# Atif-Anwer/SHMGAN

Hardware: AMD Instinct MI355X
Metric: images/sec (gen+disc train_step) (higher is better)
Workload: dtype f32; 1 GPU; SHMGAN train_step 256x256 5-view, batch 8/GPU, filter_size 64, fp32 (BASELINE configs[1]); global_batch=8, image_size=256, parallelism=dp1, losses_finite=True

## Files before the change

shmgan_amd/csrc/imgloss.hip:

```cpp
#include "common.h"

#define Y2R_V_R 1.13988303f
#define Y2R_U_G -0.394642334f
#define Y2R_V_G -0.58062185f
#define Y2R_U_B 2.03206185f

constexpr int NSUM = 19;
constexpr int WIN = SHM_SSIM_WIN;
constexpr int TILE = 16;
constexpr int HALO = TILE + WIN - 1;

struct ImgArgs {
    const float* gen_rgb;
    const float* cyc_rgb;
    const float* cyc_y;
    const float* cbcr;
    const float* orig[5];
    const float* ds[5];
    int flags;
    float style_factor;
    double* loss;
    float* dgen_y;
    float* dcyc_y;
    double* sums;
    unsigned* mm;
    float* gd;
    double* ssim_sum;
    float* gcoef;
    double* rsum;
    int* argpos;
    float* dmaps;
    int batch, s;
};

__device__ __forceinline__ unsigned f2ord(float f) {
    unsigned u = __float_as_uint(f);
    return (u & 0x80000000u) ? ~u : (u | 0x80000000u);
}
__device__ __forceinline__ float ord2f(unsigned u) {
    return __uint_as_float((u & 0x80000000u) ? (u & 0x7fffffffu) : ~u);
}

__global__ __launch_bounds__(256) void img_pass_a(const ImgArgs a) {
    const int b = blockIdx.y, B = a.batch;
    const size_t npix = (size_t)a.s * a.s;
    const float invB = 1.0f / B, inv3n = 1.0f / (3.0f * (float)npix);
    double sm[NSUM];
#pragma unroll
    for (int i = 0; i < NSUM; ++i) sm[i] = 0.0;
    float mn[10], mx[10];
#pragma unroll
    for (int i = 0; i < 10; ++i) { mn[i] = 3.0e38f; mx[i] = -3.0e38f; }

    for (size_t p = (size_t)blockIdx.x * 256 + threadIdx.x; p < npix; p += (size_t)gridDim.x * 256) {
        const size_t bp = (size_t)b * npix + p;
        const float u = a.cbcr[bp * 2], v = a.cbcr[bp * 2 + 1];
        {
            float g = 0.f;
#pragma unroll
            for (int c = 0; c < 3; ++c) {
                float d = a.gen_rgb[bp * 3 + c] - a.orig[4][bp * 3 + c];
                sm[0] += fabs((double)d);
                g += (d > 0.f) ? 1.f : (d < 0.f ? -1.f : 0.f);
            }
            a.dgen_y[bp] = 10.0f * 0.2f * invB * inv3n * g;
        }
#pragma unroll
        for (int k = 0; k < 5; ++k) {
            const size_t ip = ((size_t)k * B + b) * npix + p;
            float g = 0.f;
#pragma unroll
            for (int c = 0; c < 3; ++c) {
                float d = a.cyc_rgb[ip * 3 + c] - a.orig[k][bp * 3 + c];
                sm[1 + k] += fabs((double)d);
                g += (d > 0.f) ? 1.f : (d < 0.f ? -1.f : 0.f);
            }
            float grad = 10.0f * (k == 4 ? 10.0f : 0.2f) * invB * inv3n * g;
            const float y = a.cyc_y[ip];
            mn[k] = fminf(mn[k], fminf(y, fminf(u, v)));
            mx[k] = fmaxf(mx[k], fmaxf(y, fmaxf(u, v)));
            const float d0 = a.ds[k][bp * 3], d1 = a.ds[k][bp * 3 + 1], d2 = a.ds[k][bp * 3 + 2];
            mn[5 + k] = fminf(mn[5 + k], fminf(d0, fminf(d1, d2)));
            mx[5 + k] = fmaxf(mx[5 + k], fmaxf(d0, fmaxf(d1, d2)));
            if (k == 4) {
                const float e0 = y - a.ds[0][bp * 3], e1 = u - a.ds[0][bp * 3 + 1], e2 = v - a.ds[0][bp * 3 + 2];
                sm[6] += (double)e0 * e0 + (double)e1 * e1 + (double)e2 * e2;
                grad += 10.0f * invB * 2.0f * e0 * inv3n;
                sm[7] += (double)y * y;  sm[8] += (double)y * u;  sm[9] += (double)y * v;
                sm[10] += (double)u * u; sm[11] += (double)u * v; sm[12] += (double)v * v;
                sm[13] += (double)d0 * d0; sm[14] += (double)d0 * d1; sm[15] += (double)d0 * d2;
                sm[16] += (double)d1 * d1; sm[17] += (double)d1 * d2; sm[18] += (double)d2 * d2;
            }
            a.dcyc_y[ip] = grad;
        }
    }
#pragma unroll
    for (int i = 0; i < NSUM; ++i) {
        double s = shm_block_sum<256>(sm[i]);
        if (threadIdx.x == 0) atomicAdd(&a.sums[(size_t)b * NSUM + i], s);
    }
#pragma unroll
    for (int i = 0; i < 10; ++i) {
        float lo = shm_wave_min(mn[i]), hi = shm_wave_max(mx[i]);
        if ((threadIdx.x & 63) == 0) {
            atomicMin(&a.mm[((size_t)b * 10 + i) * 2], f2ord(lo));
            atomicMax(&a.mm[((size_t)b * 10 + i) * 2 + 1], f2ord(hi));
        }
    }
}

__global__ void img_pass_b(const ImgArgs a) {
    if (blockIdx.x != 0 || threadIdx.x != 0) return;
    const double npix = (double)a.s * a.s;
    for (int b = 0; b < a.batch; ++b) {
        const double* sm = a.sums + (size_t)b * NSUM;
        for (int i = 0; i < 6; ++i) a.loss[i] += sm[i] / (3.0 * npix);
        a.loss[16] += sm[6] / (3.0 * npix);
        double D[6];
        for (int i = 0; i < 6; ++i) D[i] = (sm[7 + i] - sm[13 + i]) / npix;
        double sq = D[0] * D[0] + D[3] * D[3] + D[5] * D[5] + 2.0 * (D[1] * D[1] + D[2] * D[2] + D[4] * D[4]);
        a.loss[17] += (double)a.style_factor * sq / 9.0;
        a.gd[b * 4 + 0] = (float)D[0];
        a.gd[b * 4 + 1] = (float)D[1];
        a.gd[b * 4 + 2] = (float)D[2];
    }
}

__global__ void img_style_grad(const ImgArgs a) {
    const size_t npix = (size_t)a.s * a.s;
    size_t idx = (size_t)blockIdx.x * blockDim.x + threadIdx.x;
    if (idx >= (size_t)a.batch * npix) return;
    const int b = (int)(idx / npix);
    const size_t ip = (size_t)4 * a.batch * npix + idx;
    const float y = a.cyc_y[ip], u = a.cbcr[idx * 2], v = a.cbcr[idx * 2 + 1];
    const float coef = 1000.0f / a.batch * 4.0f * a.style_factor / (9.0f * (float)npix);
    a.dcyc_y[ip] += coef * (a.gd[b * 4] * y + a.gd[b * 4 + 1] * u + a.gd[b * 4 + 2] * v);
}

__device__ __forceinline__ float cyc_val(const ImgArgs& a, int b, int k, int c, size_t p, size_t npix) {
    if (c == 0) return a.cyc_y[((size_t)k * a.batch + b) * npix + p];
    return a.cbcr[((size_t)b * npix + p) * 2 + (c - 1)];
}

__global__ __launch_bounds__(256) void ssim_fwd_kernel(const ImgArgs a) {
    __shared__ float xs[HALO][HALO + 1], ys[HALO][HALO + 1];
    __shared__ float hx[HALO][TILE + 1], hy[HALO][TILE + 1], hxy[HALO][TILE + 1], hsq[HALO][TILE + 1];
    __shared__ float w1[WIN];
    const int S = a.s, HO = S - WIN + 1;
    const int tiles_x = (HO + TILE - 1) / TILE;
    const int ty = blockIdx.x / tiles_x, tx = blockIdx.x % tiles_x;
    const int bk = blockIdx.y, b = bk / 5, k = bk % 5, c = blockIdx.z;
    const size_t npix = (size_t)S * S;
    const float xmn = ord2f(a.mm[((size_t)b * 10 + k) * 2]), xmx = ord2f(a.mm[((size_t)b * 10 + k) * 2 + 1]);
    const float ymn = ord2f(a.mm[((size_t)b * 10 + 5 + k) * 2]), ymx = ord2f(a.mm[((size_t)b * 10 + 5 + k) * 2 + 1]);
    const float xr = xmx > xmn ? xmx - xmn : 0.f, yr = ymx > ymn ? ymx - ymn : 0.f;
    if (threadIdx.x == 0) shm_ssim_gauss1d(w1);
    const int oy0 = ty * TILE, ox0 = tx * TILE;
    for (int i = threadIdx.x; i < HALO * HALO; i += 256) {
        int r = i / HALO, cc = i % HALO;
        int yy = oy0 + r, xx = ox0 + cc;
        float xv = 0.f, yv = 0.f;
        if (yy < S && xx < S) {
            size_t p = (size_t)yy * S + xx;
            float xraw = cyc_val(a, b, k, c, p, npix);
            float yraw = a.ds[k][((size_t)b * npix + p) * 3 + c];
            xv = xr > 0.f ? (xraw - xmn) / xr : 0.f;
            yv = yr > 0.f ? (yraw - ymn) / yr : 0.f;
        }
        xs[r][cc] = xv;
        ys[r][cc] = yv;
    }
    __syncthreads();
    for (int i = threadIdx.x; i < HALO * TILE; i += 256) {
        const int r = i / TILE, cx = i % TILE;
        float rx = 0.f, ry = 0.f, rxy = 0.f, rsq = 0.f;
        for (int j = 0; j < WIN; ++j) {
            float xv = xs[r][cx + j], yv = ys[r][cx + j], w = w1[j];
            rx += w * xv;
            ry += w * yv;
            rxy += w * xv * yv;
            rsq += w * (xv * xv + yv * yv);
        }
        hx[r][cx] = rx;
        hy[r][cx] = ry;
        hxy[r][cx] = rxy;
        hsq[r][cx] = rsq;
    }
    __syncthreads();
    const int ly = threadIdx.x / TILE, lx = threadIdx.x % TILE;
    const int oy = oy0 + ly, ox = ox0 + lx;
    double sval = 0.0;
    if (oy < HO && ox < HO) {
        float mx_ = 0.f, my_ = 0.f, exy = 0.f, esq = 0.f;
        for (int i = 0; i < WIN; ++i) {
            mx_ += w1[i] * hx[ly + i][lx];
            my_ += w1[i] * hy[ly + i][lx];
            exy += w1[i] * hxy[ly + i][lx];
            esq += w1[i] * hsq[ly + i][lx];
        }
        const float c1 = 0.0025f, c2 = 0.0225f;
        const float A1 = 2.f * mx_ * my_ + c1, B1 = mx_ * mx_ + my_ * my_ + c1;
        const float A2 = 2.f * exy - 2.f * mx_ * my_ + c2, B2 = esq - mx_ * mx_ - my_ * my_ + c2;
        const float l = A1 / B1, cs = A2 / B2;
        sval = (double)(l * cs);
        const float dmx = cs * (2.f * my_ * B1 - A1 * 2.f * mx_) / (B1 * B1) + l * (-2.f * my_ * B2 + A2 * 2.f * mx_) / (B2 * B2);
        const float dexy = l * 2.f / B2;
        const float desq = -l * A2 / (B2 * B2);
        const size_t no = (size_t)HO * HO;
        float* dm = a.dmaps + ((size_t)bk * 3 + c) * 3 * no + (size_t)oy * HO + ox;
        dm[0] = dmx;
        dm[no] = dexy;
        dm[2 * no] = desq;
    }
    sval = shm_block_sum<256>(sval);
    if (threadIdx.x == 0) atomicAdd(&a.ssim_sum[bk], sval);
}

__global__ void ssim_finalize_kernel(const ImgArgs a) {
    if (blockIdx.x != 0 || threadIdx.x != 0) return;
    const int HO = a.s - WIN + 1;
    const double cnt = 3.0 * (double)HO * HO;
    for (int b = 0; b < a.batch; ++b)
        for (int k = 0; k < 5; ++k) {
            double ssim = a.ssim_sum[b * 5 + k] / cnt;
            bool fl = (a.flags >> k) & 1;
            a.loss[6 + k] += ssim;
            double sl = fl ? 0.0 : -log((1.0 + ssim) / 2.0);
            a.loss[11 + k] += sl;
            double coef = 10.0 * (k == 4 ? 2.0 : 0.2) / a.batch;
            a.gcoef[b * 5 + k] = fl ? 0.f : (float)(coef * (-1.0 / (1.0 + ssim)) / cnt);
        }
}

__global__ __launch_bounds__(256) void ssim_bwd_kernel(const ImgArgs a) {
    __shared__ float d0[HALO][HALO + 1], d1[HALO][HALO + 1], d2[HALO][HALO + 1];
    __shared__ float h0[HALO][TILE + 1], h1[HALO][TILE + 1], h2[HALO][TILE + 1];
    __shared__ float w1[WIN];
    const int S = a.s, HO = S - WIN + 1;
    const int tiles_x = (S + TILE - 1) / TILE;
    const int ty = blockIdx.x / tiles_x, tx = blockIdx.x % tiles_x;
    const int bk = blockIdx.y, b = bk / 5, k = bk % 5, c = blockIdx.z;
    const float gco = a.gcoef[bk];
    if (gco == 0.f) return;
    const size_t npix = (size_t)S * S, no = (size_t)HO * HO;
    const float xmn = ord2f(a.mm[((size_t)b * 10 + k) * 2]), xmx = ord2f(a.mm[((size_t)b * 10 + k) * 2 + 1]);
    const float ymn = ord2f(a.mm[((size_t)b * 10 + 5 + k) * 2]), ymx = ord2f(a.mm[((size_t)b * 10 + 5 + k) * 2 + 1]);
    const float xr = xmx > xmn ? xmx - xmn : 0.f, yr = ymx > ymn ? ymx - ymn : 0.f;
    if (threadIdx.x == 0) shm_ssim_gauss1d(w1);
    const int qy0 = ty * TILE, qx0 = tx * TILE;
    const float* dm = a.dmaps + ((size_t)bk * 3 + c) * 3 * no;
    for (int i = threadIdx.x; i < HALO * HALO; i += 256) {
        int r = i / HALO, cc = i % HALO;
        int py = qy0 - (WIN - 1) + r, px = qx0 - (WIN - 1) + cc;
        float v0 = 0.f, v1 = 0.f, v2 = 0.f;
        if (py >= 0 && py < HO && px >= 0 && px < HO) {
            size_t o = (size_t)py * HO + px;
            v0 = dm[o];
            v1 = dm[no + o];
            v2 = dm[2 * no + o];
        }
        d0[r][cc] = v0;
        d1[r][cc] = v1;
        d2[r][cc] = v2;
    }
    __syncthreads();
    for (int i = threadIdx.x; i < HALO * TILE; i += 256) {
        const int rr = i / TILE, cx = i % TILE;
        float r0 = 0.f, r1 = 0.f, r2 = 0.f;
        for (int j = 0; j < WIN; ++j) {
            const int cc = cx + (WIN - 1) - j;
            const float w = w1[j];
            r0 += w * d0[rr][cc];
            r1 += w * d1[rr][cc];
            r2 += w * d2[rr][cc];
        }
        h0[rr][cx] = r0;
        h1[rr][cx] = r1;
        h2[rr][cx] = r2;
    }
    __syncthreads();
    const int ly = threadIdx.x / TILE, lx = threadIdx.x % TILE;
    const int qy = qy0 + ly, qx = qx0 + lx;
    double sdx = 0.0, sdxr = 0.0;
    if (qy < S && qx < S) {
        float g0 = 0.f, g1 = 0.f, g2 = 0.f;
        for (int i = 0; i < WIN; ++i) {
            const int rr = ly + (WIN - 1) - i;
            g0 += w1[i] * h0[rr][lx];
            g1 += w1[i] * h1[rr][lx];
            g2 += w1[i] * h2[rr][lx];
        }
        const size_t p = (size_t)qy * S + qx;
        const float xraw = cyc_val(a, b, k, c, p, npix);
        const float yraw = a.ds[k][((size_t)b * npix + p) * 3 + c];
        const float xv = xr > 0.f ? (xraw - xmn) / xr : 0.f;
        const float yv = yr > 0.f ? (yraw - ymn) / yr : 0.f;
        const float dx = gco * (g0 + yv * g1 + 2.f * xv * g2);
        sdx = (double)dx;
        sdxr = (double)dx * (double)xv;
        if (c == 0 && xr > 0.f) {
            a.dcyc_y[((size_t)k * a.batch + b) * npix + p] += dx / xr;
            if (xraw == xmn) a.argpos[bk * 2] = (int)p;
            if (xraw == xmx) a.argpos[bk * 2 + 1] = (int)p;
        }
    }
    sdx = shm_block_sum<256>(sdx);
    sdxr = shm_block_sum<256>(sdxr);
    if (threadIdx.x == 0) {
        atomicAdd(&a.rsum[bk * 2], sdx);
        atomicAdd(&a.rsum[bk * 2 + 1], sdxr);
    }
}

__global__ void ssim_minmax_kernel(const ImgArgs a) {
    int bk = blockIdx.x * blockDim.x + threadIdx.x;
    if (bk >= a.batch * 5) return;
    const int b = bk / 5, k = bk % 5;
    if (a.gcoef[bk] == 0.f) return;
    const float xmn = ord2f(a.mm[((size_t)b * 10 + k) * 2]), xmx = ord2f(a.mm[((size_t)b * 10 + k) * 2 + 1]);
    if (!(xmx > xmn)) return;
    const double inv = 1.0 / ((double)xmx - (double)xmn);
    const double sdx = a.rsum[bk * 2], sdxr = a.rsum[bk * 2 + 1];
    const size_t npix = (size_t)a.s * a.s;
    float* dy = a.dcyc_y + ((size_t)k * a.batch + b) * npix;
    const int pmin = a.argpos[bk * 2], pmax = a.argpos[bk * 2 + 1];
    if (pmin >= 0) dy[pmin] += (float)(-(sdx - sdxr) * inv);
    if (pmax >= 0) dy[pmax] += (float)(-sdxr * inv);
}

static size_t align256(size_t v) { return (v + 255) & ~(size_t)255; }

struct WsPlan {
    size_t sums, mm, gd, ssim_sum, gcoef, rsum, argpos, dmaps, total, zero_bytes;
};

static WsPlan plan_ws(int batch, int s) {
    WsPlan w;
    size_t off = 0;
    w.sums = off;     off = align256(off + (size_t)batch * NSUM * 8);
    w.ssim_sum = off; off = align256(off + (size_t)batch * 5 * 8);
    w.rsum = off;     off = align256(off + (size_t)batch * 10 * 8);
    w.gd = off;       off = align256(off + (size_t)batch * 4 * 4);
    w.gcoef = off;    off = align256(off + (size_t)batch * 5 * 4);
    w.zero_bytes = off;
    w.mm = off;       off = align256(off + (size_t)batch * 20 * 4);
    w.argpos = off;   off = align256(off + (size_t)batch * 10 * 4);
    w.dmaps = off;
    int ho = s - WIN + 1;
    off = align256(off + (size_t)batch * 5 * 3 * 3 * ho * ho * 4);
    w.total = off;
    return w;
}

extern "C" size_t shm_image_losses_workspace(int batch, int s) {
    if (s < WIN) return 0;
    return plan_ws(batch, s).total;
}

__global__ void init_mm_kernel(unsigned* mm, int n) {
    int i = blockIdx.x * blockDim.x + threadIdx.x;
    if (i < n) mm[i] = (i & 1) ? 0u : 0xffffffffu;
}

extern "C" int shm_image_losses(const float* gen_rgb, const float* cyc_rgb, const float* cyc_y, const float* cbcr,
                                const float* const* orig, const float* const* ds, int flags_mask, float style_factor,
                                double* loss, float* dgen_y, float* dcyc_y, void* ws, size_t ws_bytes, int batch, int s,
                                void* stream) {
    SHM_REQUIRE(s >= WIN, SHM_E_SHAPE, "shm_image_losses: image size %d < 11 (ssim window)", s);
    SHM_REQUIRE(batch > 0 && batch * 5 <= 65535, SHM_E_SHAPE, "shm_image_losses: bad batch %d", batch);
    WsPlan w = plan_ws(batch, s);
    SHM_REQUIRE(ws && ws_bytes >= w.total, SHM_E_WORKSPACE, "shm_image_losses: workspace %zu < %zu bytes", ws_bytes, w.total);
    hipStream_t st = (hipStream_t)stream;
    char* base = (char*)ws;
    ImgArgs a{};
    a.gen_rgb = gen_rgb;
    a.cyc_rgb = cyc_rgb;
    a.cyc_y = cyc_y;
    a.cbcr = cbcr;
    for (int i = 0; i < 5; ++i) {
        a.orig[i] = orig[i];
        a.ds[i] = ds[i];
    }
    a.flags = flags_mask;
    a.style_factor = style_factor;
    a.loss = loss;
    a.dgen_y = dgen_y;
    a.dcyc_y = dcyc_y;
    a.sums = (double*)(base + w.sums);
    a.mm = (unsigned*)(base + w.mm);
    a.gd = (float*)(base + w.gd);
    a.ssim_sum = (double*)(base + w.ssim_sum);
    a.gcoef = (float*)(base + w.gcoef);
    a.rsum = (double*)(base + w.rsum);
    a.argpos = (int*)(base + w.argpos);
    a.dmaps = (float*)(base + w.dmaps);
    a.batch = batch;
    a.s = s;

    int r = shm_zero(base, w.zero_bytes, stream);
    if (r) return r;
    r = shm_zero(loss, 32 * sizeof(double), stream);
    if (r) return r;
    hipError_t e = hipMemsetAsync(a.argpos, 0xff, (size_t)batch * 10 * 4, st);
    SHM_REQUIRE(e == hipSuccess, SHM_E_HIP, "shm_image_losses: memset: %s", hipGetErrorString(e));
    hipLaunchKernelGGL(init_mm_kernel, dim3(shm_cdiv(batch * 20, 64)), dim3(64), 0, st, a.mm, batch * 20);
    SHM_LAUNCH_CHECK("shm_image_losses(init)");

    const size_t npix = (size_t)s * s;
    const int nblk = shm_grid_cap(npix, 1024, 256);
    hipLaunchKernelGGL(img_pass_a, dim3(nblk, batch), dim3(256), 0, st, a);
    SHM_LAUNCH_CHECK("shm_image_losses(pass a)");
    hipLaunchKernelGGL(img_pass_b, dim3(1), dim3(64), 0, st, a);
    SHM_LAUNCH_CHECK("shm_image_losses(pass b)");
    hipLaunchKernelGGL(img_style_grad, dim3(shm_cdiv((long)(batch * npix), 256)), dim3(256), 0, st, a);
    SHM_LAUNCH_CHECK("shm_image_losses(style)");
    const int ho = s - WIN + 1;
    const int tf = shm_cdiv(ho, TILE), tb = shm_cdiv(s, TILE);
    hipLaunchKernelGGL(ssim_fwd_kernel, dim3(tf * tf, batch * 5, 3), dim3(256), 0, st, a);
    SHM_LAUNCH_CHECK("shm_image_losses(ssim fwd)");
    hipLaunchKernelGGL(ssim_finalize_kernel, dim3(1), dim3(64), 0, st, a);
    SHM_LAUNCH_CHECK("shm_image_losses(ssim finalize)");
    hipLaunchKernelGGL(ssim_bwd_kernel, dim3(tb * tb, batch * 5, 3), dim3(256), 0, st, a);
    SHM_LAUNCH_CHECK("shm_image_losses(ssim bwd)");
    hipLaunchKernelGGL(ssim_minmax_kernel, dim3(shm_cdiv(batch * 5, 64)), dim3(64), 0, st, a);
    SHM_LAUNCH_CHECK("shm_image_losses(minmax)");
    return SHM_OK;
}
```

Baseline: 70.13 images/sec.

## Replace atomic reductions in image losses with per-block partials and deterministic finalize

Pass A, the SSIM forward pass and the SSIM backward pass now write per-block or per-tile partial sums and min/max values to workspace instead of doing global double-precision atomics. Parallel finalize kernels (one block per batch or per batch-view) then reduce those partials. The serial single-thread loss accumulation is spread across threads of later kernels. This removes atomic contention, the workspace zeroing memset and the mm init kernel. The cost is a larger workspace and extra reads of the partial buffers, on a path that is small relative to the GAN convolutions.

Result: no change. 70.16 images/sec (median of 5 runs) (+0.0%).

```diff
diff --git a/shmgan_amd/csrc/imgloss.hip b/shmgan_amd/csrc/imgloss.hip
--- a/shmgan_amd/csrc/imgloss.hip
+++ b/shmgan_amd/csrc/imgloss.hip
@@ -25,12 +25,15 @@
     double* sums;
     unsigned* mm;
     float* gd;
-    double* ssim_sum;
     float* gcoef;
-    double* rsum;
     int* argpos;
     float* dmaps;
-    int batch, s;
+    double* pa_sums;
+    float* pa_mm;
+    double* tile_f;
+    double* tile_b;
+    double* ssim_val;
+    int batch, s, nblk;
 };
 
 __device__ __forceinline__ unsigned f2ord(float f) {
@@ -94,41 +97,77 @@
             a.dcyc_y[ip] = grad;
         }
     }
+    __shared__ float wmm[4][20];
+    const size_t slot = (size_t)b * gridDim.x + blockIdx.x;
 #pragma unroll
     for (int i = 0; i < NSUM; ++i) {
         double s = shm_block_sum<256>(sm[i]);
-        if (threadIdx.x == 0) atomicAdd(&a.sums[(size_t)b * NSUM + i], s);
+        if (threadIdx.x == 0) a.pa_sums[slot * NSUM + i] = s;
     }
 #pragma unroll
     for (int i = 0; i < 10; ++i) {
         float lo = shm_wave_min(mn[i]), hi = shm_wave_max(mx[i]);
         if ((threadIdx.x & 63) == 0) {
-            atomicMin(&a.mm[((size_t)b * 10 + i) * 2], f2ord(lo));
-            atomicMax(&a.mm[((size_t)b * 10 + i) * 2 + 1], f2ord(hi));
-        }
-    }
-}
-
-__global__ void img_pass_b(const ImgArgs a) {
-    if (blockIdx.x != 0 || threadIdx.x != 0) return;
+            wmm[threadIdx.x >> 6][2 * i] = lo;
+            wmm[threadIdx.x >> 6][2 * i + 1] = hi;
+        }
+    }
+    __syncthreads();
+    if (threadIdx.x < 20) {
+        const int i = threadIdx.x;
+        float v = wmm[0][i];
+        for (int w = 1; w < 4; ++w) v = (i & 1) ? fmaxf(v, wmm[w][i]) : fminf(v, wmm[w][i]);
+        a.pa_mm[slot * 20 + i] = v;
+    }
+}
+
+__global__ __launch_bounds__(64) void img_pass_b(const ImgArgs a) {
+    __shared__ double sm[NSUM];
+    const int b = blockIdx.x, t = threadIdx.x;
+    if (t < NSUM) {
+        const double* ps = a.pa_sums + (size_t)b * a.nblk * NSUM + t;
+        double v = 0.0;
+#pragma unroll 8
+        for (int j = 0; j < a.nblk; ++j) v += ps[(size_t)j * NSUM];
+        sm[t] = v;
+        a.sums[(size_t)b * NSUM + t] = v;
+    } else if (t >= 32 && t < 52) {
+        const int i = t - 32;
+        const float* pm = a.pa_mm + (size_t)b * a.nblk * 20 + i;
+        float v = pm[0];
+#pragma unroll 8
+        for (int j = 1; j < a.nblk; ++j) v = (i & 1) ? fmaxf(v, pm[(size_t)j * 20]) : fminf(v, pm[(size_t)j * 20]);
+        a.mm[(size_t)b * 20 + i] = f2ord(v);
+    }
+    __syncthreads();
+    if (t < 3) {
+        const double npix = (double)a.s * a.s;
+        a.gd[b * 4 + t] = (float)((sm[7 + t] - sm[13 + t]) / npix);
+    }
+}
+
+__device__ void img_loss_slot(const ImgArgs& a, int i) {
     const double npix = (double)a.s * a.s;
+    const int slot = i < 6 ? i : 10 + i;
+    double acc = a.loss[slot];
     for (int b = 0; b < a.batch; ++b) {
         const double* sm = a.sums + (size_t)b * NSUM;
-        for (int i = 0; i < 6; ++i) a.loss[i] += sm[i] / (3.0 * npix);
-        a.loss[16] += sm[6] / (3.0 * npix);
-        double D[6];
-        for (int i = 0; i < 6; ++i) D[i] = (sm[7 + i] - sm[13 + i]) / npix;
-        double sq = D[0] * D[0] + D[3] * D[3] + D[5] * D[5] + 2.0 * (D[1] * D[1] + D[2] * D[2] + D[4] * D[4]);
-        a.loss[17] += (double)a.style_factor * sq / 9.0;
-        a.gd[b * 4 + 0] = (float)D[0];
-        a.gd[b * 4 + 1] = (float)D[1];
-        a.gd[b * 4 + 2] = (float)D[2];
-    }
+        if (i < 7) {
+            acc += sm[i] / (3.0 * npix);
+        } else {
+            double D[6];
+            for (int j = 0; j < 6; ++j) D[j] = (sm[7 + j] - sm[13 + j]) / npix;
+            double sq = D[0] * D[0] + D[3] * D[3] + D[5] * D[5] + 2.0 * (D[1] * D[1] + D[2] * D[2] + D[4] * D[4]);
+            acc += (double)a.style_factor * sq / 9.0;
+        }
+    }
+    a.loss[slot] = acc;
 }
 
 __global__ void img_style_grad(const ImgArgs a) {
     const size_t npix = (size_t)a.s * a.s;
     size_t idx = (size_t)blockIdx.x * blockDim.x + threadIdx.x;
+    if (idx < 8) img_loss_slot(a, (int)idx);
     if (idx >= (size_t)a.batch * npix) return;
     const int b = (int)(idx / npix);
     const size_t ip = (size_t)4 * a.batch * npix + idx;
@@ -213,23 +252,34 @@
         dm[2 * no] = desq;
     }
     sval = shm_block_sum<256>(sval);
-    if (threadIdx.x == 0) atomicAdd(&a.ssim_sum[bk], sval);
-}
-
-__global__ void ssim_finalize_kernel(const ImgArgs a) {
-    if (blockIdx.x != 0 || threadIdx.x != 0) return;
+    if (threadIdx.x == 0) a.tile_f[((size_t)bk * 3 + c) * gridDim.x + blockIdx.x] = sval;
+}
+
+__global__ __launch_bounds__(256) void ssim_finalize_kernel(const ImgArgs a, int ntile) {
+    const int bk = blockIdx.x, k = bk % 5;
+    const double* t = a.tile_f + (size_t)bk * ntile;
+    double v = 0.0;
+    for (int j = threadIdx.x; j < ntile; j += 256) v += t[j];
+    v = shm_block_sum<256>(v);
+    if (threadIdx.x != 0) return;
     const int HO = a.s - WIN + 1;
     const double cnt = 3.0 * (double)HO * HO;
-    for (int b = 0; b < a.batch; ++b)
-        for (int k = 0; k < 5; ++k) {
-            double ssim = a.ssim_sum[b * 5 + k] / cnt;
-            bool fl = (a.flags >> k) & 1;
-            a.loss[6 + k] += ssim;
-            double sl = fl ? 0.0 : -log((1.0 + ssim) / 2.0);
-            a.loss[11 + k] += sl;
-            double coef = 10.0 * (k == 4 ? 2.0 : 0.2) / a.batch;
-            a.gcoef[b * 5 + k] = fl ? 0.f : (float)(coef * (-1.0 / (1.0 + ssim)) / cnt);
-        }
+    const double ssim = v / cnt;
+    const bool fl = (a.flags >> k) & 1;
+    a.ssim_val[bk] = ssim;
+    const double coef = 10.0 * (k == 4 ? 2.0 : 0.2) / a.batch;
+    a.gcoef[bk] = fl ? 0.f : (float)(coef * (-1.0 / (1.0 + ssim)) / cnt);
+}
+
+__device__ void ssim_loss_slots(const ImgArgs& a, int k) {
+    double s = a.loss[6 + k], l = a.loss[11 + k];
+    for (int b = 0; b < a.batch; ++b) {
+        const double ssim = a.ssim_val[b * 5 + k];
+        s += ssim;
+        l += ((a.flags >> k) & 1) ? 0.0 : -log((1.0 + ssim) / 2.0);
+    }
+    a.loss[6 + k] = s;
+    a.loss[11 + k] = l;
 }
 
 __global__ __launch_bounds__(256) void ssim_bwd_kernel(const ImgArgs a) {
@@ -307,20 +357,29 @@
     sdx = shm_block_sum<256>(sdx);
     sdxr = shm_block_sum<256>(sdxr);
     if (threadIdx.x == 0) {
-        atomicAdd(&a.rsum[bk * 2], sdx);
-        atomicAdd(&a.rsum[bk * 2 + 1], sdxr);
-    }
-}
-
-__global__ void ssim_minmax_kernel(const ImgArgs a) {
-    int bk = blockIdx.x * blockDim.x + threadIdx.x;
-    if (bk >= a.batch * 5) return;
+        const size_t nt = (size_t)3 * gridDim.x, slot = (size_t)c * gridDim.x + blockIdx.x;
+        a.tile_b[((size_t)bk * 2) * nt + slot] = sdx;
+        a.tile_b[((size_t)bk * 2 + 1) * nt + slot] = sdxr;
+    }
+}
+
+__global__ __launch_bounds__(256) void ssim_minmax_kernel(const ImgArgs a, int ntile) {
+    const int bk = blockIdx.x;
+    if (bk == 0 && threadIdx.x >= 64 && threadIdx.x < 69) ssim_loss_slots(a, threadIdx.x - 64);
     const int b = bk / 5, k = bk % 5;
     if (a.gcoef[bk] == 0.f) return;
     const float xmn = ord2f(a.mm[((size_t)b * 10 + k) * 2]), xmx = ord2f(a.mm[((size_t)b * 10 + k) * 2 + 1]);
     if (!(xmx > xmn)) return;
+    const double* t = a.tile_b + (size_t)bk * 2 * ntile;
+    double sdx = 0.0, sdxr = 0.0;
+    for (int j = threadIdx.x; j < ntile; j += 256) {
+        sdx += t[j];
+        sdxr += t[ntile + j];
+    }
+    sdx = shm_block_sum<256>(sdx);
+    sdxr = shm_block_sum<256>(sdxr);
+    if (threadIdx.x != 0) return;
     const double inv = 1.0 / ((double)xmx - (double)xmn);
-    const double sdx = a.rsum[bk * 2], sdxr = a.rsum[bk * 2 + 1];
     const size_t npix = (size_t)a.s * a.s;
     float* dy = a.dcyc_y + ((size_t)k * a.batch + b) * npix;
     const int pmin = a.argpos[bk * 2], pmax = a.argpos[bk * 2 + 1];
@@ -331,22 +390,28 @@
 static size_t align256(size_t v) { return (v + 255) & ~(size_t)255; }
 
 struct WsPlan {
-    size_t sums, mm, gd, ssim_sum, gcoef, rsum, argpos, dmaps, total, zero_bytes;
+    size_t sums, mm, gd, ssim_val, gcoef, argpos, pa_sums, pa_mm, tile_f, tile_b, dmaps, total;
+    int nblk, tf, tb;
 };
 
 static WsPlan plan_ws(int batch, int s) {
     WsPlan w;
+    const int ho = s - WIN + 1;
+    w.nblk = shm_grid_cap((size_t)s * s, 1024, 256);
+    w.tf = shm_cdiv(ho, TILE);
+    w.tb = shm_cdiv(s, TILE);
     size_t off = 0;
     w.sums = off;     off = align256(off + (size_t)batch * NSUM * 8);
-    w.ssim_sum = off; off = align256(off + (size_t)batch * 5 * 8);
-    w.rsum = off;     off = align256(off + (size_t)batch * 10 * 8);
+    w.ssim_val = off; off = align256(off + (size_t)batch * 5 * 8);
     w.gd = off;       off = align256(off + (size_t)batch * 4 * 4);
     w.gcoef = off;    off = align256(off + (size_t)batch * 5 * 4);
-    w.zero_bytes = off;
     w.mm = off;       off = align256(off + (size_t)batch * 20 * 4);
     w.argpos = off;   off = align256(off + (size_t)batch * 10 * 4);
+    w.pa_sums = off;  off = align256(off + (size_t)batch * w.nblk * NSUM * 8);
+    w.pa_mm = off;    off = align256(off + (size_t)batch * w.nblk * 20 * 4);
+    w.tile_f = off;   off = align256(off + (size_t)batch * 5 * 3 * w.tf * w.tf * 8);
+    w.tile_b = off;   off = align256(off + (size_t)batch * 5 * 2 * 3 * w.tb * w.tb * 8);
     w.dmaps = off;
-    int ho = s - WIN + 1;
     off = align256(off + (size_t)batch * 5 * 3 * 3 * ho * ho * 4);
     w.total = off;
     return w;
@@ -355,11 +420,6 @@
 extern "C" size_t shm_image_losses_workspace(int batch, int s) {
     if (s < WIN) return 0;
     return plan_ws(batch, s).total;
-}
-
-__global__ void init_mm_kernel(unsigned* mm, int n) {
-    int i = blockIdx.x * blockDim.x + threadIdx.x;
-    if (i < n) mm[i] = (i & 1) ? 0u : 0xffffffffu;
 }
 
 extern "C" int shm_image_losses(const float* gen_rgb, const float* cyc_rgb, const float* cyc_y, const float* cbcr,
@@ -389,40 +449,37 @@
     a.sums = (double*)(base + w.sums);
     a.mm = (unsigned*)(base + w.mm);
     a.gd = (float*)(base + w.gd);
-    a.ssim_sum = (double*)(base + w.ssim_sum);
+    a.ssim_val = (double*)(base + w.ssim_val);
     a.gcoef = (float*)(base + w.gcoef);
-    a.rsum = (double*)(base + w.rsum);
     a.argpos = (int*)(base + w.argpos);
+    a.pa_sums = (double*)(base + w.pa_sums);
+    a.pa_mm = (float*)(base + w.pa_mm);
+    a.tile_f = (double*)(base + w.tile_f);
+    a.tile_b = (double*)(base + w.tile_b);
     a.dmaps = (float*)(base + w.dmaps);
     a.batch = batch;
     a.s = s;
-
-    int r = shm_zero(base, w.zero_bytes, stream);
-    if (r) return r;
-    r = shm_zero(loss, 32 * sizeof(double), stream);
+    a.nblk = w.nblk;
+
+    int r = shm_zero(loss, 32 * sizeof(double), stream);
     if (r) return r;
     hipError_t e = hipMemsetAsync(a.argpos, 0xff, (size_t)batch * 10 * 4, st);
     SHM_REQUIRE(e == hipSuccess, SHM_E_HIP, "shm_image_losses: memset: %s", hipGetErrorString(e));
-    hipLaunchKernelGGL(init_mm_kernel, dim3(shm_cdiv(batch * 20, 64)), dim3(64), 0, st, a.mm, batch * 20);
-    SHM_LAUNCH_CHECK("shm_image_losses(init)");
 
     const size_t npix = (size_t)s * s;
-    const int nblk = shm_grid_cap(npix, 1024, 256);
-    hipLaunchKernelGGL(img_pass_a, dim3(nblk, batch), dim3(256), 0, st, a);
+    hipLaunchKernelGGL(img_pass_a, dim3(w.nblk, batch), dim3(256), 0, st, a);
     SHM_LAUNCH_CHECK("shm_image_losses(pass a)");
-    hipLaunchKernelGGL(img_pass_b, dim3(1), dim3(64), 0, st, a);
+    hipLaunchKernelGGL(img_pass_b, dim3(batch), dim3(64), 0, st, a);
     SHM_LAUNCH_CHECK("shm_image_losses(pass b)");
     hipLaunchKernelGGL(img_style_grad, dim3(shm_cdiv((long)(batch * npix), 256)), dim3(256), 0, st, a);
     SHM_LAUNCH_CHECK("shm_image_losses(style)");
-    const int ho = s - WIN + 1;
-    const int tf = shm_cdiv(ho, TILE), tb = shm_cdiv(s, TILE);
-    hipLaunchKernelGGL(ssim_fwd_kernel, dim3(tf * tf, batch * 5, 3), dim3(256), 0, st, a);
+    hipLaunchKernelGGL(ssim_fwd_kernel, dim3(w.tf * w.tf, batch * 5, 3), dim3(256), 0, st, a);
     SHM_LAUNCH_CHECK("shm_image_losses(ssim fwd)");
-    hipLaunchKernelGGL(ssim_finalize_kernel, dim3(1), dim3(64), 0, st, a);
+    hipLaunchKernelGGL(ssim_finalize_kernel, dim3(batch * 5), dim3(256), 0, st, a, 3 * w.tf * w.tf);
     SHM_LAUNCH_CHECK("shm_image_losses(ssim finalize)");
-    hipLaunchKernelGGL(ssim_bwd_kernel, dim3(tb * tb, batch * 5, 3), dim3(256), 0, st, a);
+    hipLaunchKernelGGL(ssim_bwd_kernel, dim3(w.tb * w.tb, batch * 5, 3), dim3(256), 0, st, a);
     SHM_LAUNCH_CHECK("shm_image_losses(ssim bwd)");
-    hipLaunchKernelGGL(ssim_minmax_kernel, dim3(shm_cdiv(batch * 5, 64)), dim3(64), 0, st, a);
+    hipLaunchKernelGGL(ssim_minmax_kernel, dim3(batch * 5), dim3(256), 0, st, a, 3 * w.tb * w.tb);
     SHM_LAUNCH_CHECK("shm_image_losses(minmax)");
     return SHM_OK;
 }
```
